# Bioinfo-Tools/PANGEA-plus

Hardware: AMD Instinct MI355X
Metric: classified reads/sec (+ HBM GB/s fraction), 150 bp vs 1 Gbp db, 1/2/4/8 GPU (higher is better)
Workload: dtype u64 (2-bit packed bases, integer scores)

## Files before the change

### pangea-plus_amd/csrc/dust.hip

```cpp
#include <type_traits>

#include "bitops.hpp"
#include "engine.hpp"

namespace pgx {

constexpr int kDustMaxT = 62, kDustLevel = 20;

__device__ __forceinline__ void dust_wave_sync()
{
	asm volatile("s_waitcnt lgkmcnt(0)" ::: "memory");
	__builtin_amdgcn_wave_barrier();
}
struct ScanLane {
	uint32_t w[64];
	uint32_t pad;
};
static_assert(sizeof(ScanLane) / 4 % 2 == 1, "odd word stride");

template <int NR> __device__ __forceinline__ uint64_t reg_window64(const uint64_t (&R)[NR], int pos)
{
	const int wi = __builtin_amdgcn_readfirstlane(pos >> 5), sh = (pos & 31) * 2;
	uint64_t lo = 0, hi = 0;
#pragma unroll
	for (int k = 0; k + 1 < NR; k++)
		if (wi == k) {
			lo = R[k];
			hi = R[k + 1];
		}
	return sh ? (lo >> sh) | (hi << (64 - sh)) : lo;
}

template <int NW>
__global__ __launch_bounds__(64) void k_dust_scan(const uint64_t *__restrict__ fwd, const uint64_t *__restrict__ amb,
						   const uint32_t *__restrict__ len, const uint32_t *__restrict__ woff, uint32_t n,
						   uint32_t *__restrict__ list, uint2 *__restrict__ range, uint32_t *__restrict__ n_list)
{
	constexpr bool REGS = NW > 0;
	constexpr int NR = REGS ? NW + 1 : 1;
	__shared__ ScanLane s_lane[64];
	uint32_t *tab = s_lane[threadIdx.x].w;
	const uint32_t at0 = blockIdx.x * 64u + threadIdx.x;
	const bool has_read = at0 < n;
	const uint32_t r = has_read ? at0 : 0u;
	const int nt = has_read ? (int)len[r] - 2 : 0;
	const uint64_t *rw = fwd + woff[r], *ra = (!REGS && amb) ? amb + woff[r] : nullptr;
	uint64_t R[NR];
	if constexpr (REGS) {
#pragma unroll
		for (int k = 0; k < NR; k++)
			R[k] = k < NW ? rw[k] : 0ull;
	}
	for (int k = 0; k < 64; k++)
		tab[k] = 0u;
	int first = -1, last = -1;
	int size = 0, start = 0, rw_pairs = 0;
	uint64_t in_w = 0, out_w = 0;
	int out_pos = -1;
	int nt_wave = nt;
	if constexpr (REGS) {
		for (int sh = 1; sh < 64; sh <<= 1) {
			const int o = __shfl_xor(nt_wave, sh);
			nt_wave = o > nt_wave ? o : nt_wave;
		}
	}
	for (int b = 0; b < nt_wave; b++) {
		int t = -1;
		if constexpr (REGS) {
			if ((b & 15) == 0)
				in_w = reg_window64(R, b);
			if (b >= kDustMaxT && ((b - kDustMaxT) & 15) == 0)
				out_w = reg_window64(R, b - kDustMaxT);
		}
		if (b < nt) {
			if constexpr (REGS) {
				t = (int)((in_w >> (2 * (b & 15))) & 63ull);
			} else {
				if ((b & 15) == 0)
					in_w = window64(rw, b);
				t = (int)(in_w & 63ull);
				in_w >>= 2;
				if (ra && (window64(ra, b) & 0x15ull))
					t = -1;
				if (t < 0) {
					for (int k = 0; k < 64; k++)
						tab[k] = 0u;
					size = rw_pairs = 0;
					start = b + 1;
				}
			}
		}
		if (t >= 0) {
			uint32_t wt = tab[t];
			int cnt = (int)(wt >> 24);
			if (size >= kDustMaxT) {
				const int ob = b - kDustMaxT;
				int s0;
				if constexpr (REGS) {
					s0 = (int)((out_w >> (2 * (ob & 15))) & 63ull);
				} else {
					if (ob != out_pos || (ob & 15) == 0) {
						out_w = window64(rw, ob);
						out_pos = ob;
					}
					s0 = (int)(out_w & 63ull);
					out_w >>= 2;
					out_pos++;
				}
				if (s0 != t) {
					const uint32_t ws = tab[s0];
					tab[s0] = ws - (1u << 24);
					rw_pairs += cnt - ((int)(ws >> 24) - 1);
					cnt++;
				}
			} else {
				size++;
				rw_pairs += cnt;
				cnt++;
			}
			if (cnt >= 5) {
				const int d = (b - (int)((wt >> 18) & 63u)) & 63;
				const int cand = b - d + 1;
				start = cand > start ? cand : start;
			}
			tab[t] = (((wt << 6) | (uint32_t)(b & 63)) & 0xFFFFFFu) | ((uint32_t)cnt << 24);
			int L = b - start + 1;
			L = L < size ? L : size;
			if (rw_pairs * 10 > L * kDustLevel) {
				first = first < 0 ? b : first;
				last = b;
			}
		}
	}
	const unsigned long long listed = __ballot(first >= 0);
	if (listed) {
		uint32_t base = 0;
		const int leader = __ffsll((unsigned long long)listed) - 1;
		if ((int)(threadIdx.x & 63) == leader)
			base = atomicAdd(n_list, (uint32_t)__popcll(listed));
		base = __shfl(base, leader);
		if (first >= 0) {
			const uint32_t at = base + (uint32_t)__popcll(listed & ((1ull << (threadIdx.x & 63)) - 1ull));
			list[at] = r;
			range[at] = make_uint2((uint32_t)first, (uint32_t)last);
		}
	}
}

__device__ __forceinline__ int dust_dpp_up(int v, int last_lane_value)
{
	return __builtin_amdgcn_update_dpp(last_lane_value, v, 0x130, 0xf, 0xf, false);
}

__global__ __launch_bounds__(64) void k_dust_perfect(const uint64_t *__restrict__ fwd, const uint64_t *__restrict__ amb,
						      const uint32_t *__restrict__ len, const uint32_t *__restrict__ woff,
						      const uint32_t *__restrict__ list, const uint2 *__restrict__ range, const uint32_t *__restrict__ n_list,
						      uint64_t *__restrict__ mask, uint8_t *__restrict__ any)
{
	__shared__ uint32_t s_up[3][64];
	const int lane = (int)(threadIdx.x & 63);
	const uint32_t n_in = *n_list;
	for (uint32_t at = blockIdx.x; at < n_in; at += gridDim.x) {
		const uint32_t r = list[at];
		const int L = (int)len[r], nt = L - 2;
		const uint64_t *rw = fwd + woff[r], *ra = amb ? amb + woff[r] : nullptr;
		uint64_t *mw = mask + woff[r];
		const int nw = (L + 63) >> 6;
		for (int w = lane; w < nw; w += 64)
			mw[w] = 0ull;
		asm volatile("s_waitcnt vmcnt(0)" ::: "memory");
		const int b_hi = (int)range[at].y < nt - 1 ? (int)range[at].y : nt - 1;
		const int a_lo = (int)range[at].x - (kDustMaxT - 1) > 0 ? (int)range[at].x - (kDustMaxT - 1) : 0;
		const int n_chunks = (b_hi - a_lo + 64) / 64;
		bool marked = false;
		for (int c = n_chunks - 1; c >= 0; c--) {
			const int a0 = a_lo + 64 * c;
			auto triplet = [&](int p) -> int {
				if (p >= nt || (ra && (window64(ra, p) & 0x15ull)))
					return -1;
				return (int)(window64(rw, p) & 63ull);
			};
			const int a = a0 + lane;
			const int ta = triplet(a), t_far = triplet(a + 64);
			const bool has_up = c + 1 < n_chunks;
			const uint32_t upP = has_up ? s_up[0][lane] : 0u, upN = has_up ? s_up[1][lane] : 0u, upQ = has_up ? s_up[2][lane] : 1u;
			dust_wave_sync();
			bool live = a <= b_hi && ta >= 0;
			int tb = ta;
			uint32_t P1 = 0, P2 = 0, Bn = 0, Bq = 1;
			uint32_t myP = 0, myN = 0, myQ = 1;
			int end = -1;
			const int l_max = b_hi - a0 + 1 < kDustMaxT ? b_hi - a0 + 1 : kDustMaxT;
			auto steps = [&](auto UP) {
			constexpr bool HAS_UP = decltype(UP)::value;
			int k_zero = 0, k_one = 1, k_none = -1;
			asm volatile("" : "+v"(k_zero), "+v"(k_one), "+v"(k_none));
			for (int l = 2; l <= l_max; l++) {
				const uint32_t nP1 = (uint32_t)dust_dpp_up((int)P1, HAS_UP ? __builtin_amdgcn_readlane((int)upP, l - 1) : k_zero);
				const uint32_t nP2 = (uint32_t)dust_dpp_up((int)P2, HAS_UP && l > 2 ? __builtin_amdgcn_readlane((int)upP, l - 2) : k_zero);
				const uint32_t nBn = (uint32_t)dust_dpp_up((int)Bn, HAS_UP ? __builtin_amdgcn_readlane((int)upN, l - 1) : k_zero);
				const uint32_t nBq = (uint32_t)dust_dpp_up((int)Bq, HAS_UP ? __builtin_amdgcn_readlane((int)upQ, l - 1) : k_one);
				tb = dust_dpp_up(tb, HAS_UP ? __builtin_amdgcn_readlane(t_far, l - 2) : k_none);
				live = live && tb >= 0 && a + l - 1 <= b_hi;
				const uint32_t P = P1 + nP1 - nP2 + (tb == ta ? 1u : 0u);
				const uint32_t q = (uint32_t)(l - 1);
				const bool up_better = __umul24(nBn, Bq) > __umul24(Bn, nBq);
				const uint32_t sn = up_better ? nBn : Bn, sq = up_better ? nBq : Bq;
				const uint32_t lhs = __umul24(sn, q), rhs = __umul24(P, sq);
				if (live && P * 10u > (uint32_t)kDustLevel * q && lhs <= rhs)
					end = a + l + 1;
				const bool sc_better = rhs > lhs;
				P2 = P1;
				P1 = live ? P : 0u;
				Bn = live ? (sc_better ? P : sn) : 0u;
				Bq = live ? (sc_better ? q : sq) : 1u;
				if (c > 0) {
					const uint32_t p0 = (uint32_t)__builtin_amdgcn_readlane((int)P1, 0), n0 = (uint32_t)__builtin_amdgcn_readlane((int)Bn, 0),
						       q0 = (uint32_t)__builtin_amdgcn_readlane((int)Bq, 0);
					const bool me = lane == l;
					myP = me ? p0 : myP;
					myN = me ? n0 : myN;
					myQ = me ? q0 : myQ;
				}
			}
			};
			if (has_up)
				steps(std::true_type{});
			else
				steps(std::false_type{});
			if (c > 0) {
				s_up[0][lane] = myP;
				s_up[1][lane] = myN;
				s_up[2][lane] = myQ;
				dust_wave_sync();
			}
			if (end >= 0) {
				marked = true;
				for (int k = a; k <= end;) {
					const int w = k >> 6, lo = k & 63;
					const int hi = (end - (w << 6)) < 63 ? end - (w << 6) : 63;
					const uint64_t bits = (hi == 63 ? ~0ull : ((2ull << hi) - 1ull)) & (~0ull << lo);
					atomicOr(reinterpret_cast<unsigned long long *>(mw + w), (unsigned long long)bits);
					k = (w + 1) << 6;
				}
			}
		}
		if (__ballot(marked) && lane == 0)
			any[r] = 1;
		asm volatile("s_waitcnt vmcnt(0)" ::: "memory");
	}
}

__global__ void k_dust_windows(const uint64_t *__restrict__ mask, const uint8_t *__restrict__ any, const uint32_t *__restrict__ len,
			       const uint32_t *__restrict__ woff, const uint32_t *__restrict__ list, const uint32_t *__restrict__ n_list,
			       uint64_t *__restrict__ win_f, uint64_t *__restrict__ win_r)
{
	const uint32_t n_in = *n_list;
	for (uint32_t at = blockIdx.x * blockDim.x + threadIdx.x; at < n_in; at += gridDim.x * blockDim.x) {
		const uint32_t r = list[at];
		if (!any[r])
			continue;
		const int L = (int)len[r];
		const uint32_t w0 = woff[r];
		const int nw = (L + 63) >> 6;
		const int n_valid = L - kWord + 1;
		auto valid_bits = [&](int w) -> uint64_t {
			const int left = n_valid - (w << 6);
			return left <= 0 ? 0ull : (left >= 64 ? ~0ull : ((1ull << left) - 1ull));
		};
		for (int w = 0; w < nw; w++) {
			uint64_t f = valid_bits(w);
			uint64_t lo = mask[w0 + w], hi = w + 1 < nw ? mask[w0 + w + 1] : 0ull;
			auto shr = [](uint64_t &a, uint64_t &b, int k) {
				a |= (a >> k) | (b << (64 - k));
				b |= b >> k;
			};
			shr(lo, hi, 1);
			shr(lo, hi, 2);
			const uint64_t l4 = lo, h4 = hi;
			shr(lo, hi, 4);
			const uint64_t l8 = lo, h8 = hi;
			shr(lo, hi, 8);
			const uint64_t d = lo | ((l8 >> 16) | (h8 << 48)) | ((l4 >> 24) | (h4 << 40));
			f &= ~d;
			win_f[w0 + w] = f;
		}
		for (int w = 0; w < nw; w++) {
			uint64_t rv = valid_bits(w);
			const int s0 = n_valid - (w << 6) - 64;
			uint64_t span;
			if (s0 >= 0) {
				const int wi = s0 >> 6, sh = s0 & 63;
				const uint64_t a = win_f[w0 + wi], b = (sh && wi + 1 < nw) ? win_f[w0 + wi + 1] : 0ull;
				span = sh ? (a >> sh) | (b << (64 - sh)) : a;
			} else if (s0 > -64) {
				span = win_f[w0] << (-s0);
			} else {
				span = 0ull;
			}
			rv = __brevll(span);
			win_r[w0 + w] = rv;
		}
	}
}

static int dust_pass(const pgx_reads *rd, DustBufs &b, hipStream_t stream)
{
	const size_t n = (size_t)rd->n;
	const size_t n_mask = (size_t)rd->n_words + 24;
	PGX_TRY(b.mask.ensure(n_mask));
	PGX_TRY(b.win_f.ensure(n_mask));
	PGX_TRY(b.win_r.ensure(n_mask));
	PGX_TRY(b.any.ensure(n));
	PGX_TRY(b.list.ensure(n));
	PGX_TRY(b.range.ensure(n));
	PGX_TRY(b.n.ensure(2));
	PGX_HIP(hipMemsetAsync(b.any.data(), 0, n, stream));
	PGX_HIP(hipMemsetAsync(b.n.data(), 0, 2 * sizeof(uint32_t), stream));
	const uint64_t *amb = rd->has_amb ? rd->d_fwd_amb.data() : (const uint64_t *)nullptr;
	const dim3 g((unsigned)((n + 63) / 64)), blk(64);
#define PGX_DUST_SCAN(NW)                                                                                                                \
	hipLaunchKernelGGL(k_dust_scan<NW>, g, blk, 0, stream, rd->d_fwd.data(), amb, rd->d_len.data(), rd->d_woff.data(), (uint32_t)n, \
			   b.list.data(), b.range.data(), b.n.data())
	if (amb || rd->max_len > 512)
		PGX_DUST_SCAN(0);
	else if (rd->max_len <= 192)
		PGX_DUST_SCAN(6);
	else if (rd->max_len <= 320)
		PGX_DUST_SCAN(10);
	else
		PGX_DUST_SCAN(16);
#undef PGX_DUST_SCAN
	const unsigned grid2 = (unsigned)std::min<size_t>(n, 256 * 32);
	hipLaunchKernelGGL(k_dust_perfect, dim3(grid2), dim3(64), 0, stream, rd->d_fwd.data(), amb, rd->d_len.data(), rd->d_woff.data(), b.list.data(),
			   b.range.data(), b.n.data(), b.mask.data(), b.any.data());
	hipLaunchKernelGGL(k_dust_windows, dim3((unsigned)std::min<size_t>((n + 127) / 128, 256 * 8)), dim3(128), 0, stream, b.mask.data(), b.any.data(),
			   rd->d_len.data(), rd->d_woff.data(), b.list.data(), b.n.data(), b.win_f.data(), b.win_r.data());
	PGX_HIP(hipGetLastError());
	return 0;
}

int reads_dust(pgx_reads *rd)
{
	const size_t n = (size_t)rd->n;
	rd->has_dust = false;
	if (n == 0)
		return 0;
	DustBufs &b = rd->dustb;
	PGX_TRY(dust_pass(rd, b, 0));
	std::vector<uint8_t> &h_any = rd->h_read_dust;
	h_any.resize(n);
	PGX_TRY(b.any.download(h_any.data(), n));
	bool some = false;
	for (size_t i = 0; i < n && !some; i++)
		some = h_any[i] != 0;
	if (!some) {
		h_any.clear();
		return 0;
	}
	rd->has_dust = true;
	return 0;
}

int reads_dust_again(const pgx_reads *rd, DustBufs &b, hipStream_t stream)
{
	if (rd->n == 0)
		return 0;
	return dust_pass(rd, b, stream);
}

int dust_read_back(const char *who, const pgx_reads *rd, const DustBufs &b, hipStream_t stream, uint8_t *any_out, uint32_t *woff_out,
		   uint64_t *mask_out, uint64_t *win_f_out, uint64_t *win_r_out, int64_t cap_words, int64_t *n_words_out)
{
	const size_t n = (size_t)rd->n, nw = (size_t)rd->n_words;
	if (n_words_out)
		*n_words_out = (int64_t)nw;
	if (woff_out)
		std::copy(rd->h_woff.begin(), rd->h_woff.begin() + (ptrdiff_t)std::min(n + 1, rd->h_woff.size()), woff_out);
	if (!any_out && !mask_out && !win_f_out && !win_r_out)
		return 0;
	if ((mask_out || win_f_out || win_r_out) && cap_words < (int64_t)nw)
		return fail(PGX_E_ARG, "%s: the word arrays hold %lld words, the batch has %lld", who, (long long)cap_words, (long long)nw);
	if (n == 0)
		return 0;
	if (b.any.n < n || b.mask.n < nw || b.win_f.n < nw || b.win_r.n < nw)
		return fail(PGX_E_ARG, "%s: no DUST pass over a batch of this size has run into these buffers", who);
	PGX_HIP(hipStreamSynchronize(stream));
	if (any_out)
		PGX_TRY(b.any.download(any_out, n));
	if (mask_out)
		PGX_TRY(b.mask.download(mask_out, nw));
	if (win_f_out)
		PGX_TRY(b.win_f.download(win_f_out, nw));
	if (win_r_out)
		PGX_TRY(b.win_r.download(win_r_out, nw));
	return 0;
}

}

extern "C" int pgx_reads_get_dust(const pgx_reads *r, uint8_t *any_out, uint32_t *woff_out, uint64_t *mask_out, uint64_t *win_f_out,
				  uint64_t *win_r_out, int64_t cap_words, int64_t *n_words_out)
{
	if (!r)
		return pgx::fail(PGX_E_ARG, "pgx_reads_get_dust: null argument");
	return pgx::dust_read_back("pgx_reads_get_dust", r, r->dustb, 0, any_out, woff_out, mask_out, win_f_out, win_r_out, cap_words, n_words_out);
}

extern "C" int pgx_reads_redo_dust(pgx_reads *r)
{
	if (!r)
		return pgx::fail(PGX_E_ARG, "pgx_reads_redo_dust: null argument");
	if (int rc = pgx::require_device())
		return rc;
	return pgx::guard("pgx_reads_redo_dust", [&]() -> int {
		const bool had = r->has_dust;
		if (int rc = pgx::reads_dust(r))
			return rc;
		if (r->has_dust != had)
			return pgx::fail(PGX_E_NODEVICE, "pgx_reads_redo_dust: the masks of the batch changed between two passes");
		return 0;
	});
}
```

### pangea-plus_amd/csrc/engine.hpp

```cpp
#pragma once
#include <memory>
#include <functional>
#include <thread>
#include <atomic>
#include <mutex>
#include <string>
#include <unordered_map>
#include <vector>

#include "common.hpp"
#include "rdp_host.hpp"

struct pgx_db {
	int64_t n_seq = 0, n_bases = 0;
	bool has_amb = false;
	bool synthetic_ids = false;
	std::vector<uint32_t> h_seq_off;
	std::vector<std::string> ids;
	std::vector<uint64_t> h_words, h_amb;

	pgx::DevBuf<uint64_t> d_words, d_amb;
	pgx::DevBuf<uint32_t> d_seq_off, d_blk_subj;
	pgx::DevBuf<uint4> d_blk_info;
	pgx::DevBuf<uint32_t> d_amb_blk;
	int index_bits = 0;
	int64_t n_postings = 0;
	std::shared_ptr<void> work;
	std::mutex search_mu;
	bool dust = true;
	bool dust_each_search = false;
	bool ungapped = false;
	pgx::DevBuf<uint32_t> d_bucket_off, d_postings;
	pgx::DevBuf<uint3> d_post_ctx;

	bool bound = false;
	std::vector<std::string> lineage;
	std::vector<std::string> token_text;
	std::unordered_map<std::string, uint32_t> token_id;
	pgx::DevBuf<uint32_t> d_subj_tok_off, d_subj_tok;
	pgx::DevBuf<int8_t> d_tok_rank;
	pgx::DevBuf<uint32_t> d_subj_pairs;
	int max_pairs = 15;
	int pair_words = 16;
	std::vector<int8_t> h_tok_rank;
	std::vector<int32_t> subj_taxid;
	std::vector<std::string> lin_text;
	pgx::DevBuf<uint32_t> d_subj_lin;
	uint32_t empty_lin = 0;
	pgx::DevBuf<uint32_t> d_node_name_tok;
	pgx::DevBuf<uint32_t> d_simrank_lut;
	pgx::DevBuf<uint32_t> d_simrank_len;
	uint32_t simrank_undef = 0, simrank_zero = 0;
	uint32_t intern(const std::string &s);
	mutable std::mutex fmt_mu;
	mutable pgx::DevBuf<unsigned char> d_id_blob, d_lin_blob;
	mutable pgx::DevBuf<uint32_t> d_id_off, d_lin_off;
	mutable bool id_blob_ready = false, lin_blob_ready = false;
};

namespace pgx {
struct DustBufs {
	DevBuf<uint64_t> win_f, win_r;
	DevBuf<uint8_t> any;
	DevBuf<uint64_t> mask;
	DevBuf<uint32_t> list, n;
	DevBuf<uint2> range;
};
}

struct pgx_reads {
	int64_t n = 0;
	int64_t first = 0;
	bool synthetic = false;
	bool has_amb = false;
	std::shared_ptr<const pgx::TextBlob> h_text;
	std::vector<uint64_t> name_off;
	std::vector<uint32_t> name_len;
	pgx::DevBuf<unsigned char> d_names;
	pgx::DevBuf<uint32_t> d_name_at;
	std::vector<uint32_t> h_len, h_woff;
	std::vector<uint8_t> h_read_amb;
	std::vector<uint8_t> h_read_dust;
	struct SearchClass {
		int amb, words;
		uint32_t off, count;
		bool listed;
		int dust;
	};
	std::vector<SearchClass> classes;
	pgx::DevBuf<uint32_t> d_class_list;
	std::vector<uint64_t> h_fwd;
	int64_t n_words = 0;
	int32_t max_len = 0;
	pgx::DevBuf<uint64_t> d_fwd, d_rc, d_fwd_amb, d_rc_amb;
	bool has_dust = false;
	pgx::DustBufs dustb;
	pgx::DevBuf<uint32_t> d_len, d_woff;
	std::unique_ptr<pgx_reads> pieces;
	pgx::DevBuf<uint32_t> d_piece_first;
	pgx::DevBuf<uint32_t> d_piece_parent;
	pgx::DevBuf<uint32_t> d_piece_qoff;
	std::string name_of(int64_t i) const;
};

struct pgx_hits {
	int64_t n_reads = 0;
	int64_t n_hits = 0;
	bool gapped = true;
	pgx::DevBuf<pgx_hit> d_hits;
	pgx::DevBuf<uint32_t> d_read_off;
	pgx::DevBuf<uint32_t> d_read_cnt;
};

struct pgx_rdp {
	int64_t n = 0;
	pgx::DevBuf<uint32_t> d_off;
	pgx::DevBuf<uint32_t> d_name;
	pgx::DevBuf<int8_t> d_rank;
	pgx::DevBuf<uint32_t> d_code;
	pgx::DevBuf<uint8_t> d_present;
	int max_trip = 8;
};

namespace pgx {


struct ReadsNames {
	const pgx_reads &rd;
	size_t size() const { return (size_t)rd.n; }
	void span(size_t i, std::string &tmp, const char **p, size_t *len) const
	{
		if (rd.synthetic) {
			tmp = rd.name_of((int64_t)i);
			*p = tmp.data();
			*len = tmp.size();
		} else {
			*p = rd.h_text->data() + rd.name_off[i];
			*len = rd.name_len[i];
		}
	}
};
struct ReadNameIndex : private ReadsNames, public NameIndexT<ReadsNames> {
	explicit ReadNameIndex(const pgx_reads &r) : ReadsNames{ r }, NameIndexT<ReadsNames>(static_cast<const ReadsNames &>(*this)) {}
};

int db_upload_and_index(pgx_db *db);
int db_build_blk_info(pgx_db *db);
void index_check(const pgx_db *db, const char *where);
int reads_from_fasta_ex(const char *path, int64_t first, int64_t count, bool fold_to_g, std::vector<uint32_t> *amb_count,
			std::unique_ptr<pgx_reads> &out);
int db_fold_amb_to_g(const pgx_db *src, std::unique_ptr<pgx_db> &out);
int db_read_host(const char *prefix, std::unique_ptr<pgx_db> &out);
int64_t fasta_count_records(const char *path);
int64_t fasta_count_records_text(const char *base, size_t len, bool *at_line_start);
int reads_from_fasta_text(std::shared_ptr<const TextBlob> text, int64_t first, int64_t count, bool fold_to_g,
			  std::vector<uint32_t> *amb_count, std::unique_ptr<pgx_reads> &out);
int db_build_index(pgx_db *db);
int choose_index_bits(int64_t n_postings);

int device_line_index(const uint8_t *d_text, uint64_t n, bool open_tail, DevBuf<uint64_t> &start, uint64_t *n_lines_out);

int rdp_from_text_device(const char *text, size_t n_bytes, const pgx_reads *reads, pgx_db *db, pgx_rdp **out);

int reads_dust(pgx_reads *rd);
int reads_dust_again(const pgx_reads *rd, DustBufs &b, hipStream_t stream);
int dust_read_back(const char *who, const pgx_reads *rd, const DustBufs &b, hipStream_t stream, uint8_t *any_out, uint32_t *woff_out,
		   uint64_t *mask_out, uint64_t *win_f_out, uint64_t *win_r_out, int64_t cap_words, int64_t *n_words_out);

struct SearchCounters {
	unsigned long long probes, postings, candidates, hits;
};
int blast_search_device(pgx_db *db, pgx_reads *reads, pgx_hits *out, pgx_stage_times *times);
int consensus_device(const pgx_db *db, const pgx_hits *hits, const pgx_rdp *rdp, pgx_consensus_rec *d_out,
		     pgx_stage_times *times);

int sort_big_reads(pgx_hit *hits, const pgx_hit *scratch, const uint32_t *read_start, const uint32_t *off, uint32_t *read_cnt,
		   const uint32_t *big_list, uint32_t n_big, bool gapped);

__host__ __device__ inline int hit_qspan(const pgx_hit &h) { return h.qend - h.qstart + 1; }
__host__ __device__ inline int hit_sspan(const pgx_hit &h) { return (h.send > h.sstart ? h.send - h.sstart : h.sstart - h.send) + 1; }
__host__ __device__ inline int hit_diffs(const pgx_hit &h)
{
	const int t = hit_qspan(h) + hit_sspan(h);
	return (t - 2 * h.score - (t & 1)) / 6;
}
__host__ __device__ inline int hit_gaps(const pgx_hit &h) { return hit_diffs(h) - (int)h.mismatch; }
__host__ __device__ inline int hit_length(const pgx_hit &h) { return (hit_qspan(h) + hit_sspan(h) + hit_gaps(h)) / 2; }

#ifdef PGX_STAGE_PROBES
#define PGX_DBG_STOP(v) ((v).dbg_stop)
#define PGX_SORT_DBG(v) ((v).dbg)
#else
#define PGX_DBG_STOP(v) 0
#define PGX_SORT_DBG(v) 0
#endif

struct DbView {
	const uint64_t *words, *amb;
	const uint32_t *seq_off, *blk_subj, *bucket_off, *postings;
	const uint4 *blk_info;
	const uint3 *post_ctx;
	const uint32_t *amb_blk;
	uint32_t n_seq;
	int64_t n_bases;
	int bits;
	int gapped;
	int deep_from;
	int dbg_stop;
};

struct ReadsView {
	const uint64_t *fwd, *rc, *fwd_amb, *rc_amb;
	const uint64_t *dustwin_f, *dustwin_r;
	const uint8_t *dust_any;
	const uint32_t *len, *woff;
	uint32_t n;
	const uint32_t *list;
};


constexpr uint32_t kFragmented = 0xFFFFFFFFu;

struct GappedWork {
	DevBuf<unsigned long long> big_list, big_list2;
	DevBuf<uint32_t> big_count;
	DevBuf<uint2> side_list;
	DevBuf<uint32_t> order;
	DevBuf<uint32_t> items, bins;
	DevBuf<uint32_t> items1;
	DevBuf<uint8_t> keys1;
};
int gapped_stage(const DbView &dv, const ReadsView &rv, pgx_hit *main_table, const uint8_t *main_key, const uint32_t *read_start,
		 const uint32_t *read_cnt, pgx_hit *ovf_table, const uint8_t *ovf_key, const unsigned long long *ovf_count, unsigned long long ovf_cap, bool long_reads,
		 unsigned long long hit_cap, int max_len, GappedWork &gw, hipStream_t stream, const unsigned long long *main_used, const uint8_t *main_reg);
constexpr int kGapDeepFrom = 320;
inline int gapped_region_shift(int64_t n_bases)
{
	int s = 0;
	while (((n_bases + 1024) >> s) > 240)
		s++;
	return s;
}

__host__ __device__ inline int pident_hundredths(int matches, int length)
{
	long long num = 10000ll * matches;
	long long q = num / length, r = num % length;
	if (2 * r > length)
		return (int)(q + 1);
	if (2 * r < length)
		return (int)q;
	double d = 100.0 * (double)matches / (double)length;
	double s = fma(d, 200.0, -(double)(2 * q + 1));
	if (s > 0)
		return (int)(q + 1);
	if (s < 0)
		return (int)q;
	return (int)(q + (q & 1));
}

}
```

Before: 122.4 million.

## Bound DUST perfect-interval search with scan-derived pair and start hints; prefetch next read

The scan kernel now also records the maximum pair count seen up to the last trigger and the first position where a triplet repeats five times, and emits them in a widened uint4 range record. The perfect kernel uses these to cap the window length (l_max) and raise the lower start bound, which shrinks the number of chunks and DPP steps per listed read. It also software-pipelines the per-read metadata loads (list, range, len, woff) one iteration ahead and moves the vmcnt wait into the chunk loop. The risk is correctness if the derived bounds are not valid upper bounds on the perfect-interval length or start, and the range buffer doubles in size.

```diff
diff --git a/pangea-plus_amd/csrc/dust.hip b/pangea-plus_amd/csrc/dust.hip
--- a/pangea-plus_amd/csrc/dust.hip
+++ b/pangea-plus_amd/csrc/dust.hip
@@ -34,7 +34,7 @@
 template <int NW>
 __global__ __launch_bounds__(64) void k_dust_scan(const uint64_t *__restrict__ fwd, const uint64_t *__restrict__ amb,
 						   const uint32_t *__restrict__ len, const uint32_t *__restrict__ woff, uint32_t n,
-						   uint32_t *__restrict__ list, uint2 *__restrict__ range, uint32_t *__restrict__ n_list)
+						   uint32_t *__restrict__ list, uint4 *__restrict__ range, uint32_t *__restrict__ n_list)
 {
 	constexpr bool REGS = NW > 0;
 	constexpr int NR = REGS ? NW + 1 : 1;
@@ -54,6 +54,7 @@
 	for (int k = 0; k < 64; k++)
 		tab[k] = 0u;
 	int first = -1, last = -1;
+	int p_max = 0, p_last = 0, e0 = -1;
 	int size = 0, start = 0, rw_pairs = 0;
 	uint64_t in_w = 0, out_w = 0;
 	int out_pos = -1;
@@ -122,13 +123,16 @@
 				const int d = (b - (int)((wt >> 18) & 63u)) & 63;
 				const int cand = b - d + 1;
 				start = cand > start ? cand : start;
+				e0 = e0 < 0 ? b : e0;
 			}
 			tab[t] = (((wt << 6) | (uint32_t)(b & 63)) & 0xFFFFFFu) | ((uint32_t)cnt << 24);
 			int L = b - start + 1;
 			L = L < size ? L : size;
+			p_max = rw_pairs > p_max ? rw_pairs : p_max;
 			if (rw_pairs * 10 > L * kDustLevel) {
 				first = first < 0 ? b : first;
 				last = b;
+				p_last = p_max;
 			}
 		}
 	}
@@ -142,7 +146,7 @@
 		if (first >= 0) {
 			const uint32_t at = base + (uint32_t)__popcll(listed & ((1ull << (threadIdx.x & 63)) - 1ull));
 			list[at] = r;
-			range[at] = make_uint2((uint32_t)first, (uint32_t)last);
+			range[at] = make_uint4((uint32_t)first, (uint32_t)last, (uint32_t)p_last, (uint32_t)e0);
 		}
 	}
 }
@@ -154,23 +158,36 @@
 
 __global__ __launch_bounds__(64) void k_dust_perfect(const uint64_t *__restrict__ fwd, const uint64_t *__restrict__ amb,
 						      const uint32_t *__restrict__ len, const uint32_t *__restrict__ woff,
-						      const uint32_t *__restrict__ list, const uint2 *__restrict__ range, const uint32_t *__restrict__ n_list,
+						      const uint32_t *__restrict__ list, const uint4 *__restrict__ range, const uint32_t *__restrict__ n_list,
 						      uint64_t *__restrict__ mask, uint8_t *__restrict__ any)
 {
 	__shared__ uint32_t s_up[3][64];
 	const int lane = (int)(threadIdx.x & 63);
 	const uint32_t n_in = *n_list;
-	for (uint32_t at = blockIdx.x; at < n_in; at += gridDim.x) {
-		const uint32_t r = list[at];
-		const int L = (int)len[r], nt = L - 2;
-		const uint64_t *rw = fwd + woff[r], *ra = amb ? amb + woff[r] : nullptr;
-		uint64_t *mw = mask + woff[r];
+	if (blockIdx.x >= n_in)
+		return;
+	uint32_t at = blockIdx.x;
+	uint32_t r = list[at];
+	uint4 rg = range[at];
+	uint32_t L_r = len[r], w_r = woff[r];
+	uint32_t r_next = list[at + gridDim.x < n_in ? at + gridDim.x : at];
+	for (;;) {
+		const uint32_t at_next = at + gridDim.x, at_after = at_next + gridDim.x;
+		const bool more = at_next < n_in;
+		const uint4 rg_next = range[more ? at_next : at];
+		const uint32_t L_next = len[r_next], w_next = woff[r_next];
+		const uint32_t r_after = list[at_after < n_in ? at_after : at];
+		const int L = (int)L_r, nt = L - 2;
+		const uint64_t *rw = fwd + w_r, *ra = amb ? amb + w_r : nullptr;
+		uint64_t *mw = mask + w_r;
 		const int nw = (L + 63) >> 6;
 		for (int w = lane; w < nw; w += 64)
 			mw[w] = 0ull;
-		asm volatile("s_waitcnt vmcnt(0)" ::: "memory");
-		const int b_hi = (int)range[at].y < nt - 1 ? (int)range[at].y : nt - 1;
-		const int a_lo = (int)range[at].x - (kDustMaxT - 1) > 0 ? (int)range[at].x - (kDustMaxT - 1) : 0;
+		const int b_hi = (int)rg.y < nt - 1 ? (int)rg.y : nt - 1;
+		const int cap = ((int)rg.z - 1) / 2 + 1 < kDustMaxT ? ((int)rg.z - 1) / 2 + 1 : kDustMaxT;
+		const int a_old = (int)rg.x - (kDustMaxT - 1), a_new = (int)rg.w - cap + 1;
+		const int a_cut = a_old > a_new ? a_old : a_new;
+		const int a_lo = a_cut > 0 ? a_cut : 0;
 		const int n_chunks = (b_hi - a_lo + 64) / 64;
 		bool marked = false;
 		for (int c = n_chunks - 1; c >= 0; c--) {
@@ -190,7 +207,7 @@
 			uint32_t P1 = 0, P2 = 0, Bn = 0, Bq = 1;
 			uint32_t myP = 0, myN = 0, myQ = 1;
 			int end = -1;
-			const int l_max = b_hi - a0 + 1 < kDustMaxT ? b_hi - a0 + 1 : kDustMaxT;
+			const int l_max = b_hi - a0 + 1 < cap ? b_hi - a0 + 1 : cap;
 			auto steps = [&](auto UP) {
 			constexpr bool HAS_UP = decltype(UP)::value;
 			int k_zero = 0, k_one = 1, k_none = -1;
@@ -234,6 +251,7 @@
 				s_up[2][lane] = myQ;
 				dust_wave_sync();
 			}
+			asm volatile("s_waitcnt vmcnt(0)" ::: "memory");
 			if (end >= 0) {
 				marked = true;
 				for (int k = a; k <= end;) {
@@ -247,7 +265,14 @@
 		}
 		if (__ballot(marked) && lane == 0)
 			any[r] = 1;
-		asm volatile("s_waitcnt vmcnt(0)" ::: "memory");
+		if (!more)
+			break;
+		at = at_next;
+		r = r_next;
+		rg = rg_next;
+		L_r = L_next;
+		w_r = w_next;
+		r_next = r_after;
 	}
 }
 
diff --git a/pangea-plus_amd/csrc/engine.hpp b/pangea-plus_amd/csrc/engine.hpp
--- a/pangea-plus_amd/csrc/engine.hpp
+++ b/pangea-plus_amd/csrc/engine.hpp
@@ -64,7 +64,7 @@
 	DevBuf<uint8_t> any;
 	DevBuf<uint64_t> mask;
 	DevBuf<uint32_t> list, n;
-	DevBuf<uint2> range;
+	DevBuf<uint4> range;
 };
 }
 
```

After: 125.4 million (median of 6 runs). +2.5%, better.
